# intuitive-robots/mdt_policy

Hardware: AMD Instinct MI355X
Metric: action-chunks/sec (10-step denoise, horizon=10) (higher is better)
Workload: dtype f32

## Files before the change

mdt_policy_amd/csrc/mdt_kernels.hip:

```cpp
#include <hip/hip_runtime.h>

#include <atomic>
#include <stdint.h>
#include <stdlib.h>

#include <mutex>
#include <vector>

#include "mdt_internal.h"

#include "mdt_device.h"

#define MDT_TILES_TIMING_OWNER
#include "mdt_tiles.h"
#include "mdt_tall.h"
#include "mdt_ws.h"
#include "mdt_mlp_split.h"

__global__ void k_pack_weight(const float* __restrict__ w, int n_rows, int K, float* __restrict__ packed,
                              int n_off, int K16) {
    const int64_t idx = (int64_t)blockIdx.x * blockDim.x + threadIdx.x;
    if (idx >= (int64_t)n_rows * K) return;
    const int n = (int)(idx / K), k = (int)(idx % K);
    const int nn = n + n_off;
// ... 305 lines not shown
    if (!active) return;
#pragma unroll
    for (int i = 0; i < MTILES; ++i) {
        const bool mok = m0 + i * 16 + (lane & 15) < a.M;
#pragma unroll
        for (int j = 0; j < NTW; ++j) {
            f32x4 v = apply_act(acc[i][j] + bias_v[j], a.act);
            if constexpr (RES) v = res_v[i][j] + (gated ? gate_v[i][j] * v : v);
            if (mok && nt0 + j < N16) st4(optr[i] + ncol[j], v);
        }
    }
}

template <int HD>
__global__ __launch_bounds__(512) void k_attn_proj_smallm(mdt_gemm_args a, const float* __restrict__ qkv, int64_t ldq, int T,
                                                         int causal, float scale, const float* __restrict__ zeros) {
    extern __shared__ __attribute__((aligned(16))) float lds[];
    __shared__ __attribute__((aligned(16))) float red[8 * 64 * 4];
    attn_proj_tile<HD, false>(a, qkv, ldq, T, causal, scale, blockIdx.x, blockIdx.y, lds, red, zeros, threadIdx.x);
}

template <int HD, int TKC>
__global__ __launch_bounds__(512) void k_attn_proj_wide(mdt_gemm_args a, mdt_attn_pro ap, int grid_n, const float* __restrict__ zeros) {
    extern __shared__ __attribute__((aligned(16))) float lds[];
    const int logical = xcd_remap(blockIdx.x, gridDim.x);
    const int by = logical / grid_n, bx = logical - by * grid_n;
    gemm_tile<2, 1, 8, PRO_ATTN, true, false, 1, 0, HD, TKC>(a, a.K, by, bx, lds, zeros, threadIdx.x, &ap);
}

template <int HD, int TKC>
__global__ __launch_bounds__(512) void k_attn_xattn(mdt_gemm_args a, mdt_attn_pro at, mdt_xapply_args x, const float* __restrict__ zeros) {
    extern __shared__ __attribute__((aligned(16))) float lds[];
    attn_xattn_tile<HD, TKC, 32>(a, at, x, xcd_remap(blockIdx.x, gridDim.x), lds, zeros, threadIdx.x);
}

static const int ZEROS_FLOATS = 65536;
static const int MAX_DEVICES = 32;
static float* g_zeros_dev[MAX_DEVICES] = {nullptr};
static thread_local float* g_zeros = nullptr;

static int current_device() {
    int dev = 0;
    if (hipGetDevice(&dev) != hipSuccess || dev < 0 || dev >= MAX_DEVICES) return 0;
    return dev;
}

static hipError_t ensure_zeros() {
    int dev = 0;
    hipError_t e = hipGetDevice(&dev);
    if (e != hipSuccess) return e;
    if (dev < 0 || dev >= MAX_DEVICES) return hipErrorInvalidDevice;
    if (g_zeros_dev[dev] == nullptr) {
        static std::mutex mu;
        std::lock_guard<std::mutex> lock(mu);
        if (g_zeros_dev[dev] == nullptr) {
            float* p = nullptr;
            e = hipMalloc((void**)&p, ZEROS_FLOATS * sizeof(float));
            if (e != hipSuccess) return e;
            e = hipMemset(p, 0, ZEROS_FLOATS * sizeof(float));
            if (e != hipSuccess) return e;
            g_zeros_dev[dev] = p;
        }
    }
    g_zeros = g_zeros_dev[dev];
    return hipSuccess;
}
// ... 299 lines not shown
    static size_t lds_attr_dev[MAX_DEVICES] = {0};
    size_t& lds_attr = lds_attr_dev[current_device()];
    if (lds > lds_attr) {
        hipError_t e = hipFuncSetAttribute((const void*)k_attn_proj_wide<HD, TKC>, hipFuncAttributeMaxDynamicSharedMemorySize, (int)lds);
        if (e != hipSuccess) return e;
        lds_attr = lds;
    }
    hipLaunchKernelGGL((k_attn_proj_wide<HD, TKC>), dim3(gn * gm), dim3(512), lds, s, p, ap, gn, g_zeros);
    return hipGetLastError();
}

hipError_t mdt_launch_attn_proj_wide(const mdt_gemm_args& p, const float* qkv, int64_t ldq, int H, int hd, int T, hipStream_t s) {
    if (!mdt_attn_proj_wide_supported(p, H, hd, T, 1, 0)) return hipErrorInvalidValue;
    hipError_t ze = ensure_zeros();
    if (ze != hipSuccess) return ze;
    mdt_attn_pro ap;
    ap.qkv = qkv; ap.ldq = ldq; ap.T = T; ap.scale = 1.0f / sqrtf((float)hd);
    const bool t10 = T <= 10;
    switch (hd) {
        case 16: return t10 ? launch_attn_proj_wide_t<16, 10>(p, ap, s) : launch_attn_proj_wide_t<16, 16>(p, ap, s);
        case 32: return t10 ? launch_attn_proj_wide_t<32, 10>(p, ap, s) : launch_attn_proj_wide_t<32, 16>(p, ap, s);
        default: return t10 ? launch_attn_proj_wide_t<48, 10>(p, ap, s) : launch_attn_proj_wide_t<48, 16>(p, ap, s);
    }
}

bool mdt_xattn_apply_supported(int D, int H, int Te, int Ta);

bool mdt_attn_xattn_supported(const mdt_gemm_args& p, const mdt_xapply_args& x, int H, int hd, int T, int causal, int rope) {
    return mdt_attn_proj_wide_supported(p, H, hd, T, causal, rope) && hd == 48 && p.N == p.K && p.ldo == p.N && x.y == p.out &&
           x.D == p.N && x.H == H && H == 8 && x.Ta == T && (int64_t)x.B * T == p.M &&
           mdt_xattn_apply_supported(x.D, x.H, x.Te, x.Ta);
}

template <int HD, int TKC>
static hipError_t launch_attn_xattn_t(const mdt_gemm_args& p, const mdt_attn_pro& at, const mdt_xapply_args& x, hipStream_t s) {
    const int D = 8 * HD;
    const size_t lds = ((size_t)16 * (D + 4) + (size_t)48 * (D + 16)) * sizeof(float);
    static bool attr_dev[MAX_DEVICES] = {false};
    bool& attr = attr_dev[current_device()];
    if (!attr) {
        hipError_t e = hipFuncSetAttribute((const void*)k_attn_xattn<HD, TKC>, hipFuncAttributeMaxDynamicSharedMemorySize, (int)lds);
        if (e != hipSuccess) return e;
        attr = true;
    }
    hipLaunchKernelGGL((k_attn_xattn<HD, TKC>), dim3(x.B), dim3(512), lds, s, p, at, x, g_zeros);
    return hipGetLastError();
}

hipError_t mdt_launch_attn_xattn(const mdt_gemm_args& p, const float* qkv, int64_t ldq, const mdt_xapply_args& x, int H, int hd,
                                 int T, hipStream_t s) {
    if (!mdt_attn_xattn_supported(p, x, H, hd, T, 1, 0) || ldq != 3 * (int64_t)p.K) return hipErrorInvalidValue;
    hipError_t ze = ensure_zeros();
    if (ze != hipSuccess) return ze;
    mdt_attn_pro at;
    at.qkv = qkv; at.ldq = ldq; at.T = T; at.scale = 1.0f / sqrtf((float)hd);
    return T <= 10 ? launch_attn_xattn_t<48, 10>(p, at, x, s) : launch_attn_xattn_t<48, 16>(p, at, x, s);
}

static thread_local std::vector<mdt_gemm_args> g_side_jobs;
static thread_local size_t g_side_next = 0;
static bool smallm_shape_ok(const mdt_gemm_args& a) {
    return a.M >= 1 && a.M <= 15 && (!a.ln || a.K <= 512) && a.batch <= 1 && a.K <= 4096 && !a.aux_mode && a.a_parts <= 1 &&
           a.N <= ZEROS_FLOATS && a.K <= ZEROS_FLOATS && !(a.N & 15) && (int64_t)a.N * a.K < ((int64_t)1 << 30);
}
static std::atomic<int> g_side_override{-1};
static std::atomic<int64_t> g_side_paired{0};
static bool side_enabled() {
    return g_side_override.load(std::memory_order_relaxed) != 0 && g_mdt_gemm_force == 0;
}
extern "C" void mdt_op_set_side_jobs(int32_t on) { g_side_override.store(on < 0 ? -1 : (on != 0)); }
extern "C" int64_t mdt_op_side_jobs_paired(void) { return g_side_paired.load(); }
hipError_t mdt_gemm_side_push(const mdt_gemm_args& a, hipStream_t s) {
    if (!side_enabled() || !smallm_shape_ok(a)) return mdt_launch_gemm(a, s);
    g_side_jobs.push_back(a);
    return hipSuccess;
}
hipError_t mdt_gemm_side_push_front(const mdt_gemm_args& a, hipStream_t s) {
    if (!side_enabled() || !smallm_shape_ok(a)) return mdt_launch_gemm(a, s);
    g_side_jobs.insert(g_side_jobs.begin() + g_side_next, a);
    return hipSuccess;
}
void mdt_gemm_side_drop() { g_side_jobs.clear(); g_side_next = 0; }
size_t mdt_gemm_side_pending() { return g_side_jobs.size() - g_side_next; }
hipError_t mdt_gemm_side_launch_front(hipStream_t s) {
    if (g_side_next >= g_side_jobs.size()) return hipSuccess;
    const mdt_gemm_args a = g_side_jobs[g_side_next];
    g_side_jobs.erase(g_side_jobs.begin() + g_side_next);
    std::vector<mdt_gemm_args> keep;
    keep.swap(g_side_jobs);
// ... 926 lines not shown
```

mdt_policy_amd/csrc/mdt_mlp_split.h:

```cpp
#pragma once
#include <hip/hip_runtime.h>
#include <stdint.h>

#include "mdt_device.h"
#include "mdt_internal.h"
#include "mdt_tiles.h"
#include "mdt_ws.h"

template <int NT, int R>
struct SplitRing {
    mdt_bf16x8 w[R][NT][3];
    __amdgpu_buffer_rsrc_t rs;
    unsigned voff[NT];
    __device__ __forceinline__ void open(const void* image, int64_t first_byte, int64_t tile_stride, int lane) {
        rs = __builtin_amdgcn_make_buffer_rsrc((void*)image, 0, 0xffffffffu, 0x00020000);
#pragma unroll
        for (int j = 0; j < NT; ++j) voff[j] = (unsigned)(first_byte + j * tile_stride) + 16u * (unsigned)lane;
    }
    __device__ __forceinline__ void request(int slot, int kk) {
#pragma unroll
        for (int j = 0; j < NT; ++j)
#pragma unroll
            for (int p = 0; p < 3; ++p)
                w[slot][j][p] = __builtin_bit_cast(mdt_bf16x8, __builtin_amdgcn_raw_buffer_load_b128(rs, voff[j], (kk * 3 + p) * 1024, 0));
    }
};

template <int NT, int K32, int R>
__device__ __forceinline__ void split_phase(SplitRing<NT, R>& ring, const char* xa, int rowb, int part, int lane, f32x4 (&acc)[2][NT]) {
    const int aoff = (lane & 15) * rowb + (lane >> 4) * 16;
    mdt_bf16x8 x1[2], x2[2], x3[2];
#pragma unroll
    for (int i = 0; i < 2; ++i) {
        const char* q = xa + aoff + i * 16 * rowb;
        x1[i] = *(const mdt_bf16x8*)q; x2[i] = *(const mdt_bf16x8*)(q + part); x3[i] = *(const mdt_bf16x8*)(q + 2 * part);
    }
#pragma unroll
    for (int kk = 0; kk < K32; ++kk) {
        const int u = kk % R, un = (kk + R - 1) % R;
        const bool nx = kk + 1 < K32;
        if (kk + R - 1 < K32) ring.request(un, kk + R - 1);
        const char* p0 = xa + aoff + (kk + 1) * 64;
        const char* p1 = p0 + 16 * rowb;
        MDT_SCHED_PIN
#pragma unroll
        for (int j = 0; j < NT; ++j) {
            acc[0][j] = __builtin_amdgcn_mfma_f32_16x16x32_bf16(ring.w[u][j][0], x3[0], acc[0][j], 0, 0, 0);
            acc[1][j] = __builtin_amdgcn_mfma_f32_16x16x32_bf16(ring.w[u][j][0], x3[1], acc[1][j], 0, 0, 0);
        }
        MDT_SCHED_PIN
        if (nx) { x3[0] = *(const mdt_bf16x8*)(p0 + 2 * part); x3[1] = *(const mdt_bf16x8*)(p1 + 2 * part); }
        MDT_SCHED_PIN
#pragma unroll
        for (int j = 0; j < NT; ++j) {
            acc[0][j] = __builtin_amdgcn_mfma_f32_16x16x32_bf16(ring.w[u][j][1], x2[0], acc[0][j], 0, 0, 0);
            acc[1][j] = __builtin_amdgcn_mfma_f32_16x16x32_bf16(ring.w[u][j][1], x2[1], acc[1][j], 0, 0, 0);
        }
#pragma unroll
        for (int j = 0; j < NT; ++j) {
            acc[0][j] = __builtin_amdgcn_mfma_f32_16x16x32_bf16(ring.w[u][j][0], x2[0], acc[0][j], 0, 0, 0);
            acc[1][j] = __builtin_amdgcn_mfma_f32_16x16x32_bf16(ring.w[u][j][0], x2[1], acc[1][j], 0, 0, 0);
        }
        MDT_SCHED_PIN
        if (nx) { x2[0] = *(const mdt_bf16x8*)(p0 + part); x2[1] = *(const mdt_bf16x8*)(p1 + part); }
        MDT_SCHED_PIN
#pragma unroll
        for (int j = 0; j < NT; ++j) {
            acc[0][j] = __builtin_amdgcn_mfma_f32_16x16x32_bf16(ring.w[u][j][2], x1[0], acc[0][j], 0, 0, 0);
            acc[1][j] = __builtin_amdgcn_mfma_f32_16x16x32_bf16(ring.w[u][j][2], x1[1], acc[1][j], 0, 0, 0);
        }
#pragma unroll
        for (int j = 0; j < NT; ++j) {
            acc[0][j] = __builtin_amdgcn_mfma_f32_16x16x32_bf16(ring.w[u][j][1], x1[0], acc[0][j], 0, 0, 0);
            acc[1][j] = __builtin_amdgcn_mfma_f32_16x16x32_bf16(ring.w[u][j][1], x1[1], acc[1][j], 0, 0, 0);
        }
#pragma unroll
        for (int j = 0; j < NT; ++j) {
            acc[0][j] = __builtin_amdgcn_mfma_f32_16x16x32_bf16(ring.w[u][j][0], x1[0], acc[0][j], 0, 0, 0);
            acc[1][j] = __builtin_amdgcn_mfma_f32_16x16x32_bf16(ring.w[u][j][0], x1[1], acc[1][j], 0, 0, 0);
        }
        MDT_SCHED_PIN
        if (nx) { x1[0] = *(const mdt_bf16x8*)p0; x1[1] = *(const mdt_bf16x8*)p1; }
        MDT_SCHED_PIN
    }
}

__host__ __device__ constexpr int mlp_split_lds_bytes(int D) {
    const int xs = 3 * 32 * (2 * D + 32), hs = 3 * 32 * (2 * 512 + 32);
    return xs > hs ? xs : hs;
}

template <int NTW2, int PRO>
__device__ __forceinline__ void mlp_split_tile(const mdt_gemm_args& f, const mdt_gemm_args& p, const char* __restrict__ w1s,
                                               const char* __restrict__ w2s, float* __restrict__ parts, int64_t part_stride, int by,
                                               int s, char* lds, const float* __restrict__ zeros, int tid) {
    constexpr int MTILES = 2, NWAVES = 8, MT = 32, HS = 512, NTW1 = 4, R = 2;
    constexpr int D = 128 * NTW2, K32a = D / 32, K32b = HS / 32;
    constexpr int ROWB1 = 2 * D + 32, PART1 = MT * ROWB1, ROWB2 = 2 * HS + 32, PART2 = MT * ROWB2;
    static_assert(NTW2 >= 1 && NTW2 <= 4, "D <= 512");
    const f32x4 zero4 = (f32x4){0.f, 0.f, 0.f, 0.f};
    const int lane = tid & 63, wave = tid >> 6;
    const int m0 = by * MT;
    const int nq = 4 * (lane >> 4);
    char* xs = lds;
    char* hs = lds;

    const int nt1 = (s * NWAVES + wave) * NTW1;
    SplitRing<NTW1, R> ring1;
    ring1.open(w1s, (int64_t)nt1 * K32a * 3072, (int64_t)K32a * 3072, lane);
#pragma unroll
    for (int u = 0; u < R - 1; ++u) ring1.request(u, u);
    f32x4 b1[NTW1];
    {
        const float* bp = f.bias != nullptr ? f.bias : zeros;
#pragma unroll
        for (int j = 0; j < NTW1; ++j) b1[j] = ldg4(bp + (nt1 + j) * 16 + nq);
    }
    gemm_stage_tile<MTILES, NWAVES, PRO, false, 1, 2, true>(f, (float*)xs, ROWB1, m0, 0, D, zeros, tid, lane, wave);
// ... 110 lines not shown
```

mdt_policy_amd/csrc/mdt_model.hip:

```cpp
#include <hip/hip_runtime.h>

#include <algorithm>
#include <cmath>
#include <cstdarg>
#include <cstdio>
#include <cstdlib>
#include <cstring>
#include <string>
#include <unordered_map>
#include <vector>

#include "mdt_internal.h"

static thread_local std::string g_err;

mdt_status mdt_fail(mdt_status st, const char* fmt, ...) {
    char buf[1024];
    va_list ap;
    va_start(ap, fmt);
    vsnprintf(buf, sizeof buf, fmt, ap);
    va_end(ap);
    g_err = buf;
    return st;
}
// ... 172 lines not shown
        attn_qkv(e.qkv, pre + ".attn");
        lin_begin(e.proj, D, D, xb);
        lin_part(e.proj, pre + ".attn.c_proj", D, 0, xb);
    };
    auto block_common_b = [&](EncBlock& e, const std::string& pre) {
        raw(e.ln2_w, pre + ".ln_2.weight", D);
        if (xb) raw(e.ln2_b, pre + ".ln_2.bias", D);
        lin_begin(e.fc, 4 * D, D, xb);
        lin_part(e.fc, pre + ".mlp.c_fc", 4 * D, 0, xb);
        lin_begin(e.proj2, D, 4 * D, xb);
        lin_part(e.proj2, pre + ".mlp.c_proj", D, 0, xb);
        if (D % 128 == 0 && D <= 512) {
            e.fc.ws = b.take((size_t)4 * D * D * 6 / 4);
            e.proj2.ws = b.take((size_t)4 * D * D * 6 / 4);
            add_extra(pre + ".mlp.c_fc.weight", (int64_t)4 * D * D, SLOT_PACK_SPLIT, (float*)e.fc.ws, 4 * D, D);
            add_extra(pre + ".mlp.c_proj.weight", (int64_t)4 * D * D, SLOT_PACK_SPLIT, (float*)e.proj2.ws, D, 4 * D);
        }
    };
    if (!fill_slots) { m->enc.assign(m->Le, EncBlock()); m->dec.assign(m->Ld, DecBlock()); }
    for (int l = 0; l < m->Le; ++l) {
        const std::string pre = P + "encoder.blocks." + std::to_string(l);
        block_common_a(m->enc[l], pre);
        block_common_b(m->enc[l], pre);
    }
    raw(m->enc_ln_w, P + "encoder.ln.weight", D);
    if (xb) raw(m->enc_ln_b, P + "encoder.ln.bias", D);

    lin_begin(m->kv_all, m->Ld * 2 * D, D, true);
    if (m->cond == COND_ADALN) lin_begin(m->mod_all, m->Ld * 6 * D, D, true);
    for (int l = 0; l < m->Ld; ++l) {
        const std::string pre = P + "decoder.blocks." + std::to_string(l);
        DecBlock& d = m->dec[l];
        block_common_a(d, pre);
        lin_part(m->kv_all, pre + ".cross_att.key", D, l * 2 * D, true);
        lin_begin(d.xq, D, D, true);
        lin_part(d.xq, pre + ".cross_att.query", D, 0, true);
        d.xq_pT = b.take((size_t)D * D);
        add_extra(pre + ".cross_att.query.weight", (int64_t)D * D, SLOT_PACK_T, d.xq_pT, D, D);
        lin_part(m->kv_all, pre + ".cross_att.value", D, l * 2 * D + D, true);
        lin_begin(d.xproj, D, D, xb);
        lin_part(d.xproj, pre + ".cross_att.c_proj", D, 0, xb);
        raw(d.ln3_w, pre + ".ln3.weight", D);
        raw(d.ln3_b, pre + ".ln3.bias", D);
        block_common_b(d, pre);
        if (m->cond == COND_ADALN) lin_part(m->mod_all, pre + ".adaLN_zero.modulation.1", 6 * D, l * 6 * D, true);
    }
    raw(m->dec_ln_w, P + "decoder.ln.weight", D);
    if (xb) raw(m->dec_ln_b, P + "decoder.ln.bias", D);
    if (c.use_proprio) {
        m->prop0_T = b.take((size_t)2 * D * c.proprio_dim);
        add_slot(P + "proprio_emb.0.weight", (int64_t)2 * D * c.proprio_dim, SLOT_TRANSPOSE, m->prop0_T, 2 * D, c.proprio_dim, 0);
        raw(m->prop0_b, P + "proprio_emb.0.bias", 2 * D);
        lin_begin(m->prop2, D, 2 * D, true);
        lin_part(m->prop2, P + "proprio_emb.2", D, 0, true);
    }
    lin_begin(m->sig1, 2 * D, D, true);
    lin_part(m->sig1, P + "sigma_emb.1", 2 * D, 0, true);
    lin_begin(m->sig3, D, 2 * D, true);
    lin_part(m->sig3, P + "sigma_emb.3", D, 0, true);
    m->Wa = b.take((size_t)D * A);
    add_slot(P + "action_emb.weight", (int64_t)D * A, SLOT_TRANSPOSE, m->Wa, D, A, 0);
    raw(m->ba, P + "action_emb.bias", D);
    if (c.linear_output) {
        raw(m->Wp, P + "action_pred.weight", (int64_t)A * D);
        raw(m->bp, P + "action_pred.bias", A);
    } else {
// ... 376 lines not shown
static int g_attn_wide_override = -1;
static int g_attn_wide_min_rows() {
    return g_attn_wide_override >= 0 ? (g_attn_wide_override == 0 ? 1 << 30 : g_attn_wide_override) : 1401;
}
extern "C" void mdt_op_set_attn_wide_min(int32_t rows) { g_attn_wide_override = rows; }

static int g_attn_xattn_min_rows() {
    return g_attn_wide_override == 0 ? 1 << 30 : 200;
}
static constexpr int64_t ATTN_XATTN_MAX_BATCH = 512;

static mdt_status run_self_attn(mdt_model* m, const EncBlock& e, const View& V, int64_t B, int T, bool causal,
                                ModRef mr, hipStream_t s, Stream in = Stream(), const mdt_xapply_args* fx = nullptr,
                                bool* fused = nullptr) {
    float* x = V.y;
    const int D = m->D, M = (int)(B * T);
    mdt_gemm_args g = gemm_args(x, D, e.qkv, V.qkv, 3 * D, M);
    g.ln = 1; g.ln_w = e.ln1_w; g.ln_b = e.ln1_b;
    g.rows_per_sample = T;
    if (in.parts > 1) {
        g.A = in.base; g.a_parts = in.parts; g.a_part_stride = in.stride; g.a_merged = x;
    }
    if (mr.mod && mr.shift >= 0) { g.mod = mr.mod; g.mod_stride = mr.stride; g.shift_off = mr.shift; g.scale_off = mr.scale; }
    LAUNCH(mdt_launch_gemm(g, s));
    mdt_gemm_args p = gemm_args(V.att, D, e.proj, x, D, M);
    p.residual = 1; p.rows_per_sample = T;
    if (mr.mod && mr.gate >= 0) { p.mod = mr.mod; p.mod_stride = mr.stride; p.gate_off = mr.gate; }
    if (B <= ATTN_PROJ_MAX_BATCH && mdt_attn_proj_supported(p, m->H, m->hd, T, m->cfg.use_rot_embed)) {
        LAUNCH(mdt_launch_attn_proj(p, V.qkv, 3 * D, m->H, m->hd, T, causal, s));
        return MDT_OK;
    }
    if (fx && fused && M >= g_attn_xattn_min_rows() && B <= ATTN_XATTN_MAX_BATCH &&
        mdt_attn_xattn_supported(p, *fx, m->H, m->hd, T, causal, m->cfg.use_rot_embed)) {
        LAUNCH(mdt_launch_attn_xattn(p, V.qkv, 3 * D, *fx, m->H, m->hd, T, s));
        *fused = true;
        return MDT_OK;
    }
    const int64_t wide_tiles = (int64_t)((M + 31) / 32) * ((D + 127) / 128);
    if (M >= g_attn_wide_min_rows() && (wide_tiles <= 256 || g_attn_wide_override > 0) &&
        mdt_attn_proj_wide_supported(p, m->H, m->hd, T, causal, m->cfg.use_rot_embed)) {
        LAUNCH(mdt_launch_attn_proj_wide(p, V.qkv, 3 * D, m->H, m->hd, T, s));
        return MDT_OK;
    }
    mdt_attn_args a;
    memset(&a, 0, sizeof a);
    a.q = V.qkv; a.ldq = 3 * D; a.k = V.qkv + D; a.v = V.qkv + 2 * D; a.ldkv = 3 * D;
    a.out = V.att; a.ldo = D; a.B = (int)B; a.H = m->H; a.hd = m->hd; a.Tq = T; a.Tk = T;
    a.causal = causal; a.rope = m->cfg.use_rot_embed;
    LAUNCH(mdt_launch_attention(a, m->rope_cos, m->rope_sin, s));
    LAUNCH(mdt_launch_gemm(p, s));
    return MDT_OK;
}

static int g_mlp_fuse_override = -1;
static int g_mlp_fuse_min_rows(bool split = false) {
    if (g_mlp_fuse_override >= 0) return g_mlp_fuse_override == 0 ? 1 << 30 : g_mlp_fuse_override;
    return split ? mdt_split_min_rows() : 1401;
}
extern "C" void mdt_op_set_mlp_fuse_min(int32_t rows) { g_mlp_fuse_override = rows; }

static bool g_trace_mlp = false;
struct TraceEv { hipEvent_t e0, e1, e2; };
static std::vector<TraceEv> g_trace_mlp_events;
static std::vector<float> g_trace_mlp_empty;
extern "C" void mdt_op_trace_mlp(int32_t enable) { g_trace_mlp = enable != 0; }
extern "C" int32_t mdt_op_trace_mlp_read(float* us, int32_t cap) {
// ... 10 lines not shown
    }
    g_trace_mlp_events.clear();
    return n;
}
extern "C" int32_t mdt_op_trace_mlp_read_empty(float* us, int32_t cap) {
    int32_t n = 0;
    for (float v : g_trace_mlp_empty)
        if (us && n < cap) us[n++] = v;
    return n;
}

__global__ void k_clock_stamp(uint64_t* __restrict__ out) {
    if (threadIdx.x == 0) {
        unsigned xcc;
        asm volatile("s_getreg_b32 %0, hwreg(HW_REG_XCC_ID)" : "=s"(xcc));
        xcc &= 7u;
        out[2 * xcc] = __builtin_amdgcn_s_memtime();
        out[2 * xcc + 1] = __builtin_amdgcn_s_memrealtime();
    }
}
extern "C" mdt_status mdt_op_clock_stamp(uint64_t* out16, void* stream) {
    if (!out16) return fail(MDT_ERR_INVALID_ARG, "mdt_op_clock_stamp: null output");
    hipLaunchKernelGGL(k_clock_stamp, dim3(64), dim3(64), 0, (hipStream_t)stream, out16);
    HIP_TRY(hipGetLastError());
    return MDT_OK;
}

static mdt_status refresh_split(mdt_model* m, hipStream_t s) {
    auto one = [&](const Lin& l) -> mdt_status {
        if (l.ws) LAUNCH(mdt_launch_split_from_packed(l.wp, l.N, l.K, l.ws, s));
        return MDT_OK;
    };
    for (const EncBlock& e : m->enc) { MDT_TRY(one(e.qkv)); MDT_TRY(one(e.fc)); MDT_TRY(one(e.proj2)); }
    for (const DecBlock& d : m->dec) { MDT_TRY(one(d.qkv)); MDT_TRY(one(d.fc)); MDT_TRY(one(d.proj2)); }
    m->split_stale = false;
    return MDT_OK;
}
static inline mdt_status split_ready(mdt_model* m, int64_t rows, hipStream_t s) {
    if (m->split_stale && mdt_mlp_split_enabled() && rows >= mdt_split_min_rows()) return refresh_split(m, s);
    return MDT_OK;
}

static mdt_status run_mlp(mdt_model* m, const EncBlock& e, const View& V, int64_t B, int T, ModRef mr, hipStream_t s,
                          Stream* out = nullptr, const mdt_xapply_args* pre_x = nullptr) {
    float* x = V.y;
    const int D = m->D, M = (int)(B * T);
    mdt_gemm_args g = gemm_args(x, D, e.fc, V.hid, 4 * D, M);
    g.ln = 1; g.ln_w = e.ln2_w; g.ln_b = e.ln2_b; g.act = MDT_ACT_GELU;
    g.rows_per_sample = T;
    if (mr.mod && mr.shift >= 0) { g.mod = mr.mod; g.mod_stride = mr.stride; g.shift_off = mr.shift; g.scale_off = mr.scale; }
    mdt_gemm_args p = gemm_args(V.hid, 4 * D, e.proj2, pre_x ? pre_x->y_out : x, D, M);
    p.residual = 1; p.rows_per_sample = T;
    if (mr.mod && mr.gate >= 0) { p.mod = mr.mod; p.mod_stride = mr.stride; p.gate_off = mr.gate; }
    if (out) *out = Stream();
    const bool split = e.fc.ws && e.proj2.ws && mdt_mlp_split_enabled() && M >= mdt_split_min_rows() && mdt_mlp_split_supported(g, p);
    if (out && !pre_x && M >= g_mlp_fuse_min_rows(split) && mdt_mlp_slices(D) >= 2 && mdt_mlp_supported(g, p)) {
        p.ldo = D;
        const int64_t stride = (int64_t)M * D;
        if (g_trace_mlp) {
            TraceEv ev;
            HIP_TRY(hipEventCreate(&ev.e0)); HIP_TRY(hipEventCreate(&ev.e1)); HIP_TRY(hipEventCreate(&ev.e2));
            HIP_TRY(hipEventRecord(ev.e0, s));
            if (split) LAUNCH(mdt_launch_mlp_split(g, p, e.fc.ws, e.proj2.ws, V.hid, stride, s));
            else LAUNCH(mdt_launch_mlp(g, p, V.hid, stride, s));
            HIP_TRY(hipEventRecord(ev.e1, s));
            HIP_TRY(hipEventRecord(ev.e2, s));
            g_trace_mlp_events.push_back(ev);
// ... 565 lines not shown
```

mdt_policy_amd/csrc/mdt_tiles.h:

```cpp
#pragma once
#include <hip/hip_runtime.h>
#include <stdint.h>

#include "mdt_internal.h"
#include "mdt_device.h"

__device__ __forceinline__ int xcd_remap(int bid, int nblocks) {
    const int q = nblocks >> 3, r = nblocks & 7, xcd = bid & 7, idx = bid >> 3;
    return (xcd < r ? xcd * (q + 1) : r * (q + 1) + (xcd - r) * q) + idx;
}

typedef unsigned u32x4_t __attribute__((ext_vector_type(4)));
template <bool COH>
struct ActLd;
template <>
struct ActLd<false> {
    const float* base;
    __device__ __forceinline__ explicit ActLd(const float* p) : base(p) {}
    __device__ __forceinline__ f32x4 ld4(int64_t off) const { return ldg4(base + off); }
    __device__ __forceinline__ float ld1(int64_t off) const { return base[off]; }
};
template <>
struct ActLd<true> {
    __amdgpu_buffer_rsrc_t rsrc;
// ... 61 lines not shown
#else
#define MDT_TS(i)
#define MDT_TS2(i)
#define MDT_TSO(off, i)
#define MDT_TS_HWID()
#endif

#define MDT_PRIO(x) if constexpr (KSTEP_PRIO) __builtin_amdgcn_s_setprio(x);
#define MDT_SCHED_PIN __builtin_amdgcn_sched_barrier(0x6);
#define MDT_KSTEP(U, KC)                                                                                  \
    {                                                                                                     \
        const int kpf = min(kg + (KC) + R - 1, K16 - 1);                                                  \
        _Pragma("unroll") for (int j = 0; j < NTW; ++j) ring[((U) + R - 1) % R][j] = wld4(wp[j] + kpf * 256); \
        MDT_SCHED_PIN                                                                                     \
        MDT_PRIO(1)                                                                                       \
        MDT_KSTEP_MFMAS(U, 0)                                                                             \
        MDT_SCHED_PIN                                                                                     \
        f32x4 avn[MTILES];  \
        _Pragma("unroll") for (int i = 0; i < MTILES; ++i) avn[i] =                                       \
            *(const f32x4*)(ap + i * 16 * stride + min((KC) + 1, nk - 1) * 16);                           \
        MDT_SCHED_PIN                                                                                     \
        MDT_KSTEP_MFMAS(U, 1)                                                                             \
        MDT_KSTEP_MFMAS(U, 2)                                                                             \
        MDT_KSTEP_MFMAS(U, 3)                                                                             \
        MDT_PRIO(0)                                                                                       \
        MDT_SCHED_PIN                                                                                     \
        _Pragma("unroll") for (int i = 0; i < MTILES; ++i) av[i] = avn[i];                                \
    }
#define MDT_KSTEP_MFMAS(U, E)                                                                             \
    _Pragma("unroll") for (int i = 0; i < MTILES; ++i) {                                                  \
        _Pragma("unroll") for (int j = 0; j < NTW; ++j) acc[i][j] =                                       \
            __builtin_amdgcn_mfma_f32_16x16x4f32(ring[(U)][j][(E)], av[i][(E)], acc[i][j], 0, 0, 0);      \
    }

template <int MTILES, int NWAVES, int PRO, bool COH, int XP = 1, int XB = 2, bool SPLIT = false>
__device__ __forceinline__ void gemm_stage_tile(const mdt_gemm_args& a, float* lds, int stride, int m0, int k0, int klen,
                                                const float* __restrict__ zeros, int tid, int lane, int wave,
                                                float* merge_out = nullptr) {
    static_assert(!SPLIT || PRO != PRO_PLAIN, "the split store belongs to the LayerNorm prologues");
    constexpr int MT = MTILES * 16;
    constexpr int NT = 64 * NWAVES;
    const f32x4 zero4 = (f32x4){0.f, 0.f, 0.f, 0.f};
    const int n4 = klen >> 2;
    const ActLd<COH> LA(a.A);
    if constexpr (PRO != PRO_PLAIN) {
        constexpr int RPW = MT / NWAVES;
        const int r0 = wave * RPW;
        int cc[2];
        bool cv[2];
#pragma unroll
        for (int p = 0; p < 2; ++p) {
            cv[p] = lane + 64 * p < n4;
            cc[p] = 4 * min(lane + 64 * p, n4 - 1);
        }
        f32x4 v[RPW][2], w[2], bb[2];
#pragma unroll
        for (int r = 0; r < RPW; ++r) {
            const int64_t m = min(m0 + r0 + r, a.M - 1);
#pragma unroll
            for (int p = 0; p < 2; ++p) v[r][p] = LA.ld4(m * a.lda + cc[p]);
        }
        if constexpr (XP > 1) {
            constexpr int HB = XB == 1 || RPW < 2 ? RPW : RPW / 2;
#pragma unroll
            for (int r0b = 0; r0b < RPW; r0b += HB) {
                f32x4 vx[XP - 1][HB][2];
// ... 201 lines not shown
            float dot = 0.f;
#pragma unroll
            for (int d = 0; d < DS; d += 4) {
                const f32x4 x = *(const f32x4*)(kp + d);
                dot = fmaf(q[d], x.x, dot); dot = fmaf(q[d + 1], x.y, dot); dot = fmaf(q[d + 2], x.z, dot); dot = fmaf(q[d + 3], x.w, dot);
            }
            dot = quad_sum(dot);
            sc[j] = j <= tq ? dot * ap.scale : -INFINITY;
            mx = fmaxf(mx, sc[j]);
        }
        float sum = 0.f;
#pragma unroll
        for (int j = 0; j < TKC; ++j) { sc[j] = expf(sc[j] - mx); sum += sc[j]; }
        const float inv = 1.0f / sum;
        float o[DS];
#pragma unroll
        for (int d = 0; d < DS; ++d) o[d] = 0.f;
#pragma unroll
        for (int j = 0; j < TKC; ++j) {
            const float pj = sc[j] * inv;
            const float* vp = vs + min(kb + min(j, tq), KVR - 1) * ST + d0;
#pragma unroll
            for (int d = 0; d < DS; d += 4) {
                const f32x4 x = *(const f32x4*)(vp + d);
                o[d] = fmaf(pj, x.x, o[d]); o[d + 1] = fmaf(pj, x.y, o[d + 1]); o[d + 2] = fmaf(pj, x.z, o[d + 2]); o[d + 3] = fmaf(pj, x.w, o[d + 3]);
            }
        }
#pragma unroll
        for (int d = 0; d < DS; d += 4)
            *(f32x4*)(xa + r * stride + hh * HHD + d0 + d) = valid ? (f32x4){o[d], o[d + 1], o[d + 2], o[d + 3]} : zero4;
    }
}

template <int HD, int TKC, class F>
__device__ __forceinline__ void attn_sample_tile(const mdt_attn_pro& ap, float* xa, int stride, int m0, float* scratch, int tid,
                                                 F after_loads) {
    constexpr int D = 8 * HD, R4 = 3 * D / 4, ST3 = 3 * D + 16;
    constexpr int NL = (TKC * R4 + 511) / 512;
    const f32x4 zero4 = (f32x4){0.f, 0.f, 0.f, 0.f};
    const int T = ap.T, total = T * R4;
    const f32x4* src = (const f32x4*)(ap.qkv + (int64_t)m0 * (3 * D));
    f32x4 t[NL];
#pragma unroll
    for (int u = 0; u < NL; ++u) t[u] = src[min(tid + 512 * u, total - 1)];
    after_loads();
    {
        int rr = tid / R4, c = tid - rr * R4;
#pragma unroll
        for (int u = 0; u < NL; ++u) {
            if (tid + 512 * u < total) *(f32x4*)(scratch + rr * ST3 + 4 * c) = t[u];
            c += 512 % R4; rr += 512 / R4;
            if (c >= R4) { c -= R4; ++rr; }
        }
    }
    __syncthreads();
    constexpr int KH = HD / 16;
    const int lane = tid & 63, h = tid >> 6, m = lane & 15, g = lane >> 4;
    const int rc = min(m, T - 1);
    f32x4 sc = zero4;
    {
        const float* qp = scratch + rc * ST3 + h * HD + 4 * g;
        const float* kp = qp + D;
        f32x4 kf[KH], qf[KH];
#pragma unroll
        for (int kc = 0; kc < KH; ++kc) { kf[kc] = *(const f32x4*)(kp + 16 * kc); qf[kc] = *(const f32x4*)(qp + 16 * kc); }
#pragma unroll
        for (int kc = 0; kc < KH; ++kc)
#pragma unroll
            for (int e = 0; e < 4; ++e) sc = __builtin_amdgcn_mfma_f32_16x16x4f32(kf[kc][e], qf[kc][e], sc, 0, 0, 0);
    }
    float vt[KH][4];
#pragma unroll
    for (int e = 0; e < 4; ++e) {
        const float* vp = scratch + min(4 * g + e, T - 1) * ST3 + 2 * D + h * HD + m;
#pragma unroll
        for (int nt = 0; nt < KH; ++nt) vt[nt][e] = vp[16 * nt];
    }
    f32x4 pr;
    {
        float mx = -INFINITY;
        bool vis[4];
#pragma unroll
        for (int e = 0; e < 4; ++e) {
            vis[e] = 4 * g + e <= rc;
            sc[e] = vis[e] ? sc[e] * ap.scale : -INFINITY;
            mx = fmaxf(mx, sc[e]);
        }
        mx = xrow_max(mx);
        float sum = 0.f;
#pragma unroll
        for (int e = 0; e < 4; ++e) { pr[e] = vis[e] ? expf(sc[e] - mx) : 0.f; sum += pr[e]; }
        const float inv = 1.0f / xrow_sum(sum);
        pr = pr * inv;
    }
    const bool valid = m < T;
#pragma unroll
    for (int nt = 0; nt < KH; ++nt) {
        f32x4 o = zero4;
#pragma unroll
        for (int e = 0; e < 4; ++e) o = __builtin_amdgcn_mfma_f32_16x16x4f32(vt[nt][e], pr[e], o, 0, 0, 0);
        *(f32x4*)(xa + m * stride + h * HD + 16 * nt + 4 * g) = valid ? o : zero4;
    }
}

template <int MTILES, int NTW, int NWAVES, int PRO, bool RES, bool COH, int XP = 1, int GLU = 0, int AHD = 48, int ATKC = 16>
__device__ __forceinline__ void gemm_tile(const mdt_gemm_args& a, int kchunk, int by, int bx, float* lds,
                                          const float* __restrict__ zeros, int tid, const mdt_attn_pro* ap = nullptr) {
    MDT_TS(0)
    MDT_TS_HWID()
    constexpr int MT = MTILES * 16;
    constexpr bool KSTEP_PRIO = false;
    constexpr int R = NTW == 1 ? 6 : (NTW == 2 ? 4 : 3);
    const f32x4 zero4 = (f32x4){0.f, 0.f, 0.f, 0.f};
    const int lane = tid & 63, wave = tid >> 6;
    const int m0 = by * MT;
    const int N16 = a.N >> 4, K16 = a.K >> 4;
    const int nt0 = (bx * NWAVES + wave) * NTW;
    const bool active = nt0 < N16;
    const int stride = kchunk + 4;
    const ActLd<COH> LO(a.out);

    WStream wp[NTW];
#pragma unroll
    for (int j = 0; j < NTW; ++j) {
        const int nt = min(nt0 + j, N16 - 1);
        wp[j] = wstream(a.Wp, (int64_t)nt * K16 * 256 + lane * 4);
    }
    f32x4 ring[R][NTW];
#pragma unroll
    for (int u = 0; u < R - 1; ++u)
#pragma unroll
        for (int j = 0; j < NTW; ++j) ring[u][j] = wld4(wp[j] + min(u, K16 - 1) * 256);

    f32x4 acc[MTILES][NTW];
// ... 996 lines not shown
        if (nk > 2) mx = fmaxf(mx, sc.z);
        if (nk > 3) mx = fmaxf(mx, sc.w);
        f32x4 e;
        e.x = expf(sc.x - mx);
        e.y = nk > 1 ? expf(sc.y - mx) : 0.f;
        e.z = nk > 2 ? expf(sc.z - mx) : 0.f;
        e.w = nk > 3 ? expf(sc.w - mx) : 0.f;
        const float inv = 1.0f / ((e.x + e.y) + (e.z + e.w));
        *(f32x4*)(prob + t * PS + 4 * h) = t < Ta ? e * inv : zero4;
    }
    __syncthreads();
    {
        const float* pp = prob + (lane & 15) * PS + 4 * (lane >> 4);
        f32x4 pv[KP16];
#pragma unroll
        for (int kc = 0; kc < KP16; ++kc) pv[kc] = *(const f32x4*)(pp + kc * 16);
        float* yb = (a.y_out != nullptr ? a.y_out : a.y) + yoff + (int64_t)(lane & 15) * D;
#pragma unroll
        for (int j = 0; j < NTWMAX; ++j)
            if (j < NTW) {
                f32x4 acc = zero4;
#pragma unroll
                for (int kc = 0; kc < KP16; ++kc)
#pragma unroll
                    for (int e = 0; e < 4; ++e) acc = __builtin_amdgcn_mfma_f32_16x16x4f32(q.wf[j][kc][e], pv[kc][e], acc, 0, 0, 0);
                const f32x4 yn = yold[j] + (q.bo[j] + acc);
                if constexpr (OL) *(f32x4*)(yo + (lane & 15) * yos + (wave * NTW + j) * 16 + nq) = yn;
                if ((lane & 15) < Ta && wr) st4(yb + (wave * NTW + j) * 16 + nq, yn);
            }
    }
    if constexpr (YL) { MDT_TS(6) } else { MDT_TS(4) }
}

template <int HD, int TKC, int NPP>
__device__ __forceinline__ void attn_xattn_tile(const mdt_gemm_args& a, const mdt_attn_pro& at, const mdt_xapply_args& x, int b,
                                                float* lds, const float* __restrict__ zeros, int tid) {
    constexpr int MTILES = 1, NTW = HD / 16, D = 8 * HD, K16 = D / 16;
    constexpr bool KSTEP_PRIO = false;
    constexpr int R = NTW == 1 ? 6 : (NTW == 2 ? 4 : 3);
    MDT_TS(0)
    MDT_TS_HWID()
    const f32x4 zero4 = (f32x4){0.f, 0.f, 0.f, 0.f};
    const int lane = tid & 63, wave = tid >> 6;
    const int T = at.T, m0 = b * T;
    constexpr int stride = D + 4;
    float* xa = lds;
    float* scr = xa + 16 * stride;
    float* yl = scr;
    float* xscr = scr + 16 * stride;

    const int nt0 = wave * NTW;
    WStream wp[NTW];
#pragma unroll
    for (int j = 0; j < NTW; ++j) wp[j] = wstream(a.Wp, (int64_t)(nt0 + j) * K16 * 256 + lane * 4);
    f32x4 ring[R][NTW];
    f32x4 acc[MTILES][NTW];
#pragma unroll
    for (int j = 0; j < NTW; ++j) acc[0][j] = zero4;
    const int nq = 4 * (lane >> 4);
    const bool gated = a.gate_off >= 0;
    int ncol[NTW];
    f32x4 bias_v[NTW], gate_v[NTW], res_v[NTW];
    mdt_xattn_req<NPP, D> xq;

    attn_sample_tile<HD, TKC>(at, xa, stride, m0, scr, tid, [&]() {
#pragma unroll
        for (int u = 0; u < R - 1; ++u)
#pragma unroll
            for (int j = 0; j < NTW; ++j) ring[u][j] = wld4(wp[j] + min(u, K16 - 1) * 256);
        const float* biasp = a.bias != nullptr ? a.bias : zeros;
        const int m = min(m0 + min(lane & 15, T - 1), a.M - 1);
        const float* gp = zeros;
        if (gated) gp = a.mod + a.gate_off + (a.mod_stride == 0 ? 0 : (int64_t)(m / a.rows_per_sample) * a.mod_stride);
#pragma unroll
        for (int j = 0; j < NTW; ++j) {
            ncol[j] = (nt0 + j) * 16 + nq;
            bias_v[j] = ldg4(biasp + ncol[j]);
            gate_v[j] = ldg4(gp + ncol[j]);
            res_v[j] = ldg4(a.out + (int64_t)m * a.ldo + ncol[j]);
        }
    });
    MDT_TS(1)
    __syncthreads();
    MDT_TS(2)
    xattn_request_u<NPP, D, D>(x, b, tid, xq);

    {
        int kg = 0;
        const int nk = K16;
        const float* ap = xa + (lane & 15) * stride + 4 * (lane >> 4);
        f32x4 av[MTILES];
        av[0] = *(const f32x4*)ap;
        int kc = 0;
        for (; kc + R <= nk; kc += R) {
#pragma unroll
            for (int u = 0; u < R; ++u) MDT_KSTEP(u, kc + u)
        }
        if (kc < nk) {
            const int rem = nk - kc;
#pragma unroll
            for (int u = 0; u < R - 1; ++u)
                if (u < rem) MDT_KSTEP(u, kc + u)
        }
        (void)kg;
    }
    MDT_TS(3)
    xattn_request_wf<NPP, D, D>(x, b, tid, xq);
    xattn_request_vec<NPP, D, D>(x, zeros, tid, xq);
#pragma unroll
    for (int j = 0; j < NTW; ++j) {
        f32x4 v = acc[0][j] + bias_v[j];
        v = res_v[j] + (gated ? gate_v[j] * v : v);
        *(f32x4*)(yl + (lane & 15) * stride + ncol[j]) = v;
    }
    __syncthreads();
    MDT_TS(4)
    xattn_tile<NPP, false, true, D, D>(x, b, xscr, zeros, tid, yl, stride, &xq);
}
```

Before: 74960.

## Use split-bf16 MFMA path for attention output projection in fused xattn kernel

Adds a split-bf16 variant of the fused attention/cross-attention kernel. The output projection weights are pre-packed into a 3-part bf16 image, and the attention output is written to LDS as three bf16 parts, so the projection can use 16x16x32 bf16 MFMAs emulating f32 instead of the f32 16x16x4 MFMAs. The SplitRing and split_phase helpers move into the shared tiles header and are generalised over the M-tile count. The change adds weight-packing memory and extra MFMA terms, and carries small numerical differences from the split emulation.

```diff
diff --git a/mdt_policy_amd/csrc/mdt_kernels.hip b/mdt_policy_amd/csrc/mdt_kernels.hip
--- a/mdt_policy_amd/csrc/mdt_kernels.hip
+++ b/mdt_policy_amd/csrc/mdt_kernels.hip
@@ -361,6 +361,11 @@
 __global__ __launch_bounds__(512) void k_attn_xattn(mdt_gemm_args a, mdt_attn_pro at, mdt_xapply_args x, const float* __restrict__ zeros) {
     extern __shared__ __attribute__((aligned(16))) float lds[];
     attn_xattn_tile<HD, TKC, 32>(a, at, x, xcd_remap(blockIdx.x, gridDim.x), lds, zeros, threadIdx.x);
+}
+template <int HD, int TKC>
+__global__ __launch_bounds__(512) void k_attn_xattn_split(mdt_gemm_args a, mdt_attn_pro at, mdt_xapply_args x, const float* __restrict__ zeros) {
+    extern __shared__ __attribute__((aligned(16))) float lds[];
+    attn_xattn_tile<HD, TKC, 32, true>(a, at, x, xcd_remap(blockIdx.x, gridDim.x), lds, zeros, threadIdx.x);
 }
 
 static const int ZEROS_FLOATS = 65536;
@@ -726,18 +731,19 @@
            mdt_xattn_apply_supported(x.D, x.H, x.Te, x.Ta);
 }
 
-template <int HD, int TKC>
+template <int HD, int TKC, bool SPLIT>
 static hipError_t launch_attn_xattn_t(const mdt_gemm_args& p, const mdt_attn_pro& at, const mdt_xapply_args& x, hipStream_t s) {
-    const int D = 8 * HD;
-    const size_t lds = ((size_t)16 * (D + 4) + (size_t)48 * (D + 16)) * sizeof(float);
+    const size_t lds = attn_xattn_lds_bytes(8 * HD, SPLIT);
+    const void* k = SPLIT ? (const void*)k_attn_xattn_split<HD, TKC> : (const void*)k_attn_xattn<HD, TKC>;
     static bool attr_dev[MAX_DEVICES] = {false};
     bool& attr = attr_dev[current_device()];
     if (!attr) {
-        hipError_t e = hipFuncSetAttribute((const void*)k_attn_xattn<HD, TKC>, hipFuncAttributeMaxDynamicSharedMemorySize, (int)lds);
+        hipError_t e = hipFuncSetAttribute(k, hipFuncAttributeMaxDynamicSharedMemorySize, (int)lds);
         if (e != hipSuccess) return e;
         attr = true;
     }
-    hipLaunchKernelGGL((k_attn_xattn<HD, TKC>), dim3(x.B), dim3(512), lds, s, p, at, x, g_zeros);
+    if constexpr (SPLIT) hipLaunchKernelGGL((k_attn_xattn_split<HD, TKC>), dim3(x.B), dim3(512), lds, s, p, at, x, g_zeros);
+    else hipLaunchKernelGGL((k_attn_xattn<HD, TKC>), dim3(x.B), dim3(512), lds, s, p, at, x, g_zeros);
     return hipGetLastError();
 }
 
@@ -748,7 +754,9 @@
     if (ze != hipSuccess) return ze;
     mdt_attn_pro at;
     at.qkv = qkv; at.ldq = ldq; at.T = T; at.scale = 1.0f / sqrtf((float)hd);
-    return T <= 10 ? launch_attn_xattn_t<48, 10>(p, at, x, s) : launch_attn_xattn_t<48, 16>(p, at, x, s);
+    if (p.Wp_split != nullptr && mdt_mlp_split_enabled())
+        return T <= 10 ? launch_attn_xattn_t<48, 10, true>(p, at, x, s) : launch_attn_xattn_t<48, 16, true>(p, at, x, s);
+    return T <= 10 ? launch_attn_xattn_t<48, 10, false>(p, at, x, s) : launch_attn_xattn_t<48, 16, false>(p, at, x, s);
 }
 
 static thread_local std::vector<mdt_gemm_args> g_side_jobs;
diff --git a/mdt_policy_amd/csrc/mdt_mlp_split.h b/mdt_policy_amd/csrc/mdt_mlp_split.h
--- a/mdt_policy_amd/csrc/mdt_mlp_split.h
+++ b/mdt_policy_amd/csrc/mdt_mlp_split.h
@@ -6,84 +6,6 @@
 #include "mdt_internal.h"
 #include "mdt_tiles.h"
 #include "mdt_ws.h"
-
-template <int NT, int R>
-struct SplitRing {
-    mdt_bf16x8 w[R][NT][3];
-    __amdgpu_buffer_rsrc_t rs;
-    unsigned voff[NT];
-    __device__ __forceinline__ void open(const void* image, int64_t first_byte, int64_t tile_stride, int lane) {
-        rs = __builtin_amdgcn_make_buffer_rsrc((void*)image, 0, 0xffffffffu, 0x00020000);
-#pragma unroll
-        for (int j = 0; j < NT; ++j) voff[j] = (unsigned)(first_byte + j * tile_stride) + 16u * (unsigned)lane;
-    }
-    __device__ __forceinline__ void request(int slot, int kk) {
-#pragma unroll
-        for (int j = 0; j < NT; ++j)
-#pragma unroll
-            for (int p = 0; p < 3; ++p)
-                w[slot][j][p] = __builtin_bit_cast(mdt_bf16x8, __builtin_amdgcn_raw_buffer_load_b128(rs, voff[j], (kk * 3 + p) * 1024, 0));
-    }
-};
-
-template <int NT, int K32, int R>
-__device__ __forceinline__ void split_phase(SplitRing<NT, R>& ring, const char* xa, int rowb, int part, int lane, f32x4 (&acc)[2][NT]) {
-    const int aoff = (lane & 15) * rowb + (lane >> 4) * 16;
-    mdt_bf16x8 x1[2], x2[2], x3[2];
-#pragma unroll
-    for (int i = 0; i < 2; ++i) {
-        const char* q = xa + aoff + i * 16 * rowb;
-        x1[i] = *(const mdt_bf16x8*)q; x2[i] = *(const mdt_bf16x8*)(q + part); x3[i] = *(const mdt_bf16x8*)(q + 2 * part);
-    }
-#pragma unroll
-    for (int kk = 0; kk < K32; ++kk) {
-        const int u = kk % R, un = (kk + R - 1) % R;
-        const bool nx = kk + 1 < K32;
-        if (kk + R - 1 < K32) ring.request(un, kk + R - 1);
-        const char* p0 = xa + aoff + (kk + 1) * 64;
-        const char* p1 = p0 + 16 * rowb;
-        MDT_SCHED_PIN
-#pragma unroll
-        for (int j = 0; j < NT; ++j) {
-            acc[0][j] = __builtin_amdgcn_mfma_f32_16x16x32_bf16(ring.w[u][j][0], x3[0], acc[0][j], 0, 0, 0);
-            acc[1][j] = __builtin_amdgcn_mfma_f32_16x16x32_bf16(ring.w[u][j][0], x3[1], acc[1][j], 0, 0, 0);
-        }
-        MDT_SCHED_PIN
-        if (nx) { x3[0] = *(const mdt_bf16x8*)(p0 + 2 * part); x3[1] = *(const mdt_bf16x8*)(p1 + 2 * part); }
-        MDT_SCHED_PIN
-#pragma unroll
-        for (int j = 0; j < NT; ++j) {
-            acc[0][j] = __builtin_amdgcn_mfma_f32_16x16x32_bf16(ring.w[u][j][1], x2[0], acc[0][j], 0, 0, 0);
-            acc[1][j] = __builtin_amdgcn_mfma_f32_16x16x32_bf16(ring.w[u][j][1], x2[1], acc[1][j], 0, 0, 0);
-        }
-#pragma unroll
-        for (int j = 0; j < NT; ++j) {
-            acc[0][j] = __builtin_amdgcn_mfma_f32_16x16x32_bf16(ring.w[u][j][0], x2[0], acc[0][j], 0, 0, 0);
-            acc[1][j] = __builtin_amdgcn_mfma_f32_16x16x32_bf16(ring.w[u][j][0], x2[1], acc[1][j], 0, 0, 0);
-        }
-        MDT_SCHED_PIN
-        if (nx) { x2[0] = *(const mdt_bf16x8*)(p0 + part); x2[1] = *(const mdt_bf16x8*)(p1 + part); }
-        MDT_SCHED_PIN
-#pragma unroll
-        for (int j = 0; j < NT; ++j) {
-            acc[0][j] = __builtin_amdgcn_mfma_f32_16x16x32_bf16(ring.w[u][j][2], x1[0], acc[0][j], 0, 0, 0);
-            acc[1][j] = __builtin_amdgcn_mfma_f32_16x16x32_bf16(ring.w[u][j][2], x1[1], acc[1][j], 0, 0, 0);
-        }
-#pragma unroll
-        for (int j = 0; j < NT; ++j) {
-            acc[0][j] = __builtin_amdgcn_mfma_f32_16x16x32_bf16(ring.w[u][j][1], x1[0], acc[0][j], 0, 0, 0);
-            acc[1][j] = __builtin_amdgcn_mfma_f32_16x16x32_bf16(ring.w[u][j][1], x1[1], acc[1][j], 0, 0, 0);
-        }
-#pragma unroll
-        for (int j = 0; j < NT; ++j) {
-            acc[0][j] = __builtin_amdgcn_mfma_f32_16x16x32_bf16(ring.w[u][j][0], x1[0], acc[0][j], 0, 0, 0);
-            acc[1][j] = __builtin_amdgcn_mfma_f32_16x16x32_bf16(ring.w[u][j][0], x1[1], acc[1][j], 0, 0, 0);
-        }
-        MDT_SCHED_PIN
-        if (nx) { x1[0] = *(const mdt_bf16x8*)p0; x1[1] = *(const mdt_bf16x8*)p1; }
-        MDT_SCHED_PIN
-    }
-}
 
 __host__ __device__ constexpr int mlp_split_lds_bytes(int D) {
     const int xs = 3 * 32 * (2 * D + 32), hs = 3 * 32 * (2 * 512 + 32);
diff --git a/mdt_policy_amd/csrc/mdt_model.hip b/mdt_policy_amd/csrc/mdt_model.hip
--- a/mdt_policy_amd/csrc/mdt_model.hip
+++ b/mdt_policy_amd/csrc/mdt_model.hip
@@ -228,6 +228,10 @@
         const std::string pre = P + "decoder.blocks." + std::to_string(l);
         DecBlock& d = m->dec[l];
         block_common_a(d, pre);
+        if (D % 128 == 0 && D <= 512) {
+            d.proj.ws = b.take((size_t)D * D * 6 / 4);
+            add_extra(pre + ".attn.c_proj.weight", (int64_t)D * D, SLOT_PACK_SPLIT, (float*)d.proj.ws, D, D);
+        }
         lin_part(m->kv_all, pre + ".cross_att.key", D, l * 2 * D, true);
         lin_begin(d.xq, D, D, true);
         lin_part(d.xq, pre + ".cross_att.query", D, 0, true);
@@ -670,6 +674,7 @@
     }
     if (fx && fused && M >= g_attn_xattn_min_rows() && B <= ATTN_XATTN_MAX_BATCH &&
         mdt_attn_xattn_supported(p, *fx, m->H, m->hd, T, causal, m->cfg.use_rot_embed)) {
+        p.Wp_split = e.proj.ws && mdt_mlp_split_enabled() && M >= mdt_split_min_rows() ? e.proj.ws : nullptr;
         LAUNCH(mdt_launch_attn_xattn(p, V.qkv, 3 * D, *fx, m->H, m->hd, T, s));
         *fused = true;
         return MDT_OK;
@@ -746,7 +751,7 @@
         return MDT_OK;
     };
     for (const EncBlock& e : m->enc) { MDT_TRY(one(e.qkv)); MDT_TRY(one(e.fc)); MDT_TRY(one(e.proj2)); }
-    for (const DecBlock& d : m->dec) { MDT_TRY(one(d.qkv)); MDT_TRY(one(d.fc)); MDT_TRY(one(d.proj2)); }
+    for (const DecBlock& d : m->dec) { MDT_TRY(one(d.qkv)); MDT_TRY(one(d.proj)); MDT_TRY(one(d.fc)); MDT_TRY(one(d.proj2)); }
     m->split_stale = false;
     return MDT_OK;
 }
diff --git a/mdt_policy_amd/csrc/mdt_tiles.h b/mdt_policy_amd/csrc/mdt_tiles.h
--- a/mdt_policy_amd/csrc/mdt_tiles.h
+++ b/mdt_policy_amd/csrc/mdt_tiles.h
@@ -117,6 +117,95 @@
         _Pragma("unroll") for (int j = 0; j < NTW; ++j) acc[i][j] =                                       \
             __builtin_amdgcn_mfma_f32_16x16x4f32(ring[(U)][j][(E)], av[i][(E)], acc[i][j], 0, 0, 0);      \
     }
+
+template <int NT, int R>
+struct SplitRing {
+    mdt_bf16x8 w[R][NT][3];
+    __amdgpu_buffer_rsrc_t rs;
+    unsigned voff[NT];
+    __device__ __forceinline__ void open(const void* image, int64_t first_byte, int64_t tile_stride, int lane) {
+        rs = __builtin_amdgcn_make_buffer_rsrc((void*)image, 0, 0xffffffffu, 0x00020000);
+#pragma unroll
+        for (int j = 0; j < NT; ++j) voff[j] = (unsigned)(first_byte + j * tile_stride) + 16u * (unsigned)lane;
+    }
+    __device__ __forceinline__ void request(int slot, int kk) {
+#pragma unroll
+        for (int j = 0; j < NT; ++j)
+#pragma unroll
+            for (int p = 0; p < 3; ++p)
+                w[slot][j][p] = __builtin_bit_cast(mdt_bf16x8, __builtin_amdgcn_raw_buffer_load_b128(rs, voff[j], (kk * 3 + p) * 1024, 0));
+    }
+};
+
+template <int NT, int K32, int R, int MT = 2>
+__device__ __forceinline__ void split_phase(SplitRing<NT, R>& ring, const char* xa, int rowb, int part, int lane, f32x4 (&acc)[MT][NT]) {
+    const int aoff = (lane & 15) * rowb + (lane >> 4) * 16;
+    mdt_bf16x8 x1[MT], x2[MT], x3[MT];
+#pragma unroll
+    for (int i = 0; i < MT; ++i) {
+        const char* q = xa + aoff + i * 16 * rowb;
+        x1[i] = *(const mdt_bf16x8*)q; x2[i] = *(const mdt_bf16x8*)(q + part); x3[i] = *(const mdt_bf16x8*)(q + 2 * part);
+    }
+#pragma unroll
+    for (int kk = 0; kk < K32; ++kk) {
+        const int u = kk % R, un = (kk + R - 1) % R;
+        const bool nx = kk + 1 < K32;
+        if (kk + R - 1 < K32) ring.request(un, kk + R - 1);
+        const char* p0 = xa + aoff + (kk + 1) * 64;
+        MDT_SCHED_PIN
+#pragma unroll
+        for (int j = 0; j < NT; ++j) {
+#pragma unroll
+            for (int i = 0; i < MT; ++i)
+                acc[i][j] = __builtin_amdgcn_mfma_f32_16x16x32_bf16(ring.w[u][j][0], x3[i], acc[i][j], 0, 0, 0);
+        }
+        MDT_SCHED_PIN
+        if (nx)
+#pragma unroll
+            for (int i = 0; i < MT; ++i) x3[i] = *(const mdt_bf16x8*)(p0 + i * 16 * rowb + 2 * part);
+        MDT_SCHED_PIN
+#pragma unroll
+        for (int j = 0; j < NT; ++j) {
+#pragma unroll
+            for (int i = 0; i < MT; ++i)
+                acc[i][j] = __builtin_amdgcn_mfma_f32_16x16x32_bf16(ring.w[u][j][1], x2[i], acc[i][j], 0, 0, 0);
+        }
+#pragma unroll
+        for (int j = 0; j < NT; ++j) {
+#pragma unroll
+            for (int i = 0; i < MT; ++i)
+                acc[i][j] = __builtin_amdgcn_mfma_f32_16x16x32_bf16(ring.w[u][j][0], x2[i], acc[i][j], 0, 0, 0);
+        }
+        MDT_SCHED_PIN
+        if (nx)
+#pragma unroll
+            for (int i = 0; i < MT; ++i) x2[i] = *(const mdt_bf16x8*)(p0 + i * 16 * rowb + part);
+        MDT_SCHED_PIN
+#pragma unroll
+        for (int j = 0; j < NT; ++j) {
+#pragma unroll
+            for (int i = 0; i < MT; ++i)
+                acc[i][j] = __builtin_amdgcn_mfma_f32_16x16x32_bf16(ring.w[u][j][2], x1[i], acc[i][j], 0, 0, 0);
+        }
+#pragma unroll
+        for (int j = 0; j < NT; ++j) {
+#pragma unroll
+            for (int i = 0; i < MT; ++i)
+                acc[i][j] = __builtin_amdgcn_mfma_f32_16x16x32_bf16(ring.w[u][j][1], x1[i], acc[i][j], 0, 0, 0);
+        }
+#pragma unroll
+        for (int j = 0; j < NT; ++j) {
+#pragma unroll
+            for (int i = 0; i < MT; ++i)
+                acc[i][j] = __builtin_amdgcn_mfma_f32_16x16x32_bf16(ring.w[u][j][0], x1[i], acc[i][j], 0, 0, 0);
+        }
+        MDT_SCHED_PIN
+        if (nx)
+#pragma unroll
+            for (int i = 0; i < MT; ++i) x1[i] = *(const mdt_bf16x8*)(p0 + i * 16 * rowb);
+        MDT_SCHED_PIN
+    }
+}
 
 template <int MTILES, int NWAVES, int PRO, bool COH, int XP = 1, int XB = 2, bool SPLIT = false>
 __device__ __forceinline__ void gemm_stage_tile(const mdt_gemm_args& a, float* lds, int stride, int m0, int k0, int klen,
@@ -384,7 +473,7 @@
     }
 }
 
-template <int HD, int TKC, class F>
+template <int HD, int TKC, bool SPLIT = false, class F>
 __device__ __forceinline__ void attn_sample_tile(const mdt_attn_pro& ap, float* xa, int stride, int m0, float* scratch, int tid,
                                                  F after_loads) {
     constexpr int D = 8 * HD, R4 = 3 * D / 4, ST3 = 3 * D + 16;
@@ -451,7 +540,16 @@
         f32x4 o = zero4;
 #pragma unroll
         for (int e = 0; e < 4; ++e) o = __builtin_amdgcn_mfma_f32_16x16x4f32(vt[nt][e], pr[e], o, 0, 0, 0);
-        *(f32x4*)(xa + m * stride + h * HD + 16 * nt + 4 * g) = valid ? o : zero4;
+        if constexpr (SPLIT) {
+            mdt_bf16x4 p1, p2, p3;
+            split3_bf16(valid ? o : zero4, p1, p2, p3);
+            char* q = (char*)xa + split_slot(m, h * HD + 16 * nt + 4 * g, stride);
+            *(mdt_bf16x4*)q = p1;
+            *(mdt_bf16x4*)(q + 16 * stride) = p2;
+            *(mdt_bf16x4*)(q + 32 * stride) = p3;
+        } else {
+            *(f32x4*)(xa + m * stride + h * HD + 16 * nt + 4 * g) = valid ? o : zero4;
+        }
     }
 }
 
@@ -1514,12 +1612,16 @@
     if constexpr (YL) { MDT_TS(6) } else { MDT_TS(4) }
 }
 
-template <int HD, int TKC, int NPP>
+__host__ __device__ constexpr int attn_xattn_lds_bytes(int D, bool split) {
+    return (split ? 3 * 16 * (2 * D + 32) : 16 * (D + 4) * 4) + 48 * (D + 16) * 4;
+}
+template <int HD, int TKC, int NPP, bool SPLIT = false>
 __device__ __forceinline__ void attn_xattn_tile(const mdt_gemm_args& a, const mdt_attn_pro& at, const mdt_xapply_args& x, int b,
                                                 float* lds, const float* __restrict__ zeros, int tid) {
     constexpr int MTILES = 1, NTW = HD / 16, D = 8 * HD, K16 = D / 16;
     constexpr bool KSTEP_PRIO = false;
     constexpr int R = NTW == 1 ? 6 : (NTW == 2 ? 4 : 3);
+    constexpr int K32 = D / 32, RS = 2, ROWB = 2 * D + 32;
     MDT_TS(0)
     MDT_TS_HWID()
     const f32x4 zero4 = (f32x4){0.f, 0.f, 0.f, 0.f};
@@ -1527,15 +1629,20 @@
     const int T = at.T, m0 = b * T;
     constexpr int stride = D + 4;
     float* xa = lds;
-    float* scr = xa + 16 * stride;
+    float* scr = xa + (SPLIT ? 3 * 16 * ROWB / 4 : 16 * stride);
     float* yl = scr;
     float* xscr = scr + 16 * stride;
 
     const int nt0 = wave * NTW;
     WStream wp[NTW];
-#pragma unroll
-    for (int j = 0; j < NTW; ++j) wp[j] = wstream(a.Wp, (int64_t)(nt0 + j) * K16 * 256 + lane * 4);
     f32x4 ring[R][NTW];
+    SplitRing<NTW, RS> sring;
+    if constexpr (SPLIT) {
+        sring.open(a.Wp_split, (int64_t)nt0 * K32 * 3072, (int64_t)K32 * 3072, lane);
+    } else {
+#pragma unroll
+        for (int j = 0; j < NTW; ++j) wp[j] = wstream(a.Wp, (int64_t)(nt0 + j) * K16 * 256 + lane * 4);
+    }
     f32x4 acc[MTILES][NTW];
 #pragma unroll
     for (int j = 0; j < NTW; ++j) acc[0][j] = zero4;
@@ -1545,11 +1652,16 @@
     f32x4 bias_v[NTW], gate_v[NTW], res_v[NTW];
     mdt_xattn_req<NPP, D> xq;
 
-    attn_sample_tile<HD, TKC>(at, xa, stride, m0, scr, tid, [&]() {
-#pragma unroll
-        for (int u = 0; u < R - 1; ++u)
-#pragma unroll
-            for (int j = 0; j < NTW; ++j) ring[u][j] = wld4(wp[j] + min(u, K16 - 1) * 256);
+    attn_sample_tile<HD, TKC, SPLIT>(at, xa, SPLIT ? ROWB : stride, m0, scr, tid, [&]() {
+        if constexpr (SPLIT) {
+#pragma unroll
+            for (int u = 0; u < RS - 1; ++u) sring.request(u, u);
+        } else {
+#pragma unroll
+            for (int u = 0; u < R - 1; ++u)
+#pragma unroll
+                for (int j = 0; j < NTW; ++j) ring[u][j] = wld4(wp[j] + min(u, K16 - 1) * 256);
+        }
         const float* biasp = a.bias != nullptr ? a.bias : zeros;
         const int m = min(m0 + min(lane & 15, T - 1), a.M - 1);
         const float* gp = zeros;
@@ -1567,7 +1679,9 @@
     MDT_TS(2)
     xattn_request_u<NPP, D, D>(x, b, tid, xq);
 
-    {
+    if constexpr (SPLIT) {
+        split_phase<NTW, K32, RS, MTILES>(sring, (const char*)xa, ROWB, 16 * ROWB, lane, acc);
+    } else {
         int kg = 0;
         const int nk = K16;
         const float* ap = xa + (lane & 15) * stride + 4 * (lane >> 4);
```

After: 75760, median of 6. 1.01x the previous value.
